# Image-Processing-Systems-Laboratory/DeepInPainting

Measured on AMD Instinct MI355X. Metric: train images/sec at 256x256, batch 8/GPU, 1/2/4/8 MI355X; IPSR layer ms, higher is better.
Workload: dtype f32; 1 GPU; BASELINE config 2: 256x256 synthetic images, 128x128 centre mask (M=256 of N=1024 feature positions), batch 8/GPU, fp32, full IPSR training step; global_batch=8, parallelism=dp1, dropout=True, conv_math=fp32, vgg16=seeded random init (no pretrained weights offline)

## Files before the change

### deepinpainting_amd/csrc/winograd.hip

```cpp
#include <type_traits>

#include "ipsr_common.h"

namespace ipsr {

typedef float f32x16 __attribute__((ext_vector_type(16)));
typedef const __attribute__((address_space(1))) void* gptr_t;
typedef __attribute__((address_space(3))) void* lptr_t;

constexpr int WG_BM = 128, WG_BN = 128, WG_BK = 16, WG_NBUF = 4, WG_THREADS = 256;

struct WinoSplit {
    int nsplit, sps, xi_split, nsplit_t, sps_t;
    int nxi = 36;
    __host__ __device__ int slabs() const { return xi_split >= nxi ? nsplit : (xi_split <= 0 ? nsplit_t : (nsplit > nsplit_t ? nsplit : nsplit_t)); }
    __host__ __device__ int of(int xi) const { return xi < xi_split ? nsplit : nsplit_t; }
    __host__ __device__ int head_xi() const { return xi_split < nxi ? xi_split : nxi; }
    __host__ int workgroups(int tiles_per_xi) const { return tiles_per_xi * (head_xi() * nsplit + (nxi - head_xi()) * nsplit_t); }
};

__device__ __forceinline__ void wino_load_sum(const float* __restrict__ M, const WinoSplit sp, size_t plane, size_t off, float m[6][6])
{
#pragma unroll
    for (int i = 0; i < 6; ++i)
// ... 1246 lines not shown
}

template <int IS, bool TMAJOR, int MODE, typename TIN>
__global__ void __launch_bounds__(256) wino5_window_kernel(const TIN* __restrict__ x, int B, int C, int H, int Wd, int nphase, int TY, int TX,
                                                           int Tp, int Cp, void* __restrict__ V, int remap)
{
    __shared__ __attribute__((aligned(16))) unsigned char smem[op_smem_bytes<TMAJOR, MODE>()];
    const int Ctot = nphase * C;
    const OpIdx ix = op_index<TMAJOR, MODE>(!TMAJOR && remap != 0);
    const int t = ix.t, cc = ix.c;
    if (!TMAJOR && MODE == 0 && t >= Tp) return;
    const int T = B * TY * TX;
    const bool live = t < T && cc < Ctot;
    int b = 0, ty = 0, tx = 0, ph = 0, c = 0;
    if (live) { b = t / (TY * TX); const int rem = t - b * TY * TX; ty = rem / TX; tx = rem - ty * TX; ph = cc / C; c = cc - ph * C; }
    const int offy = nphase == 4 ? (ph >> 1) - 1 : -1, offx = nphase == 4 ? (ph & 1) - 1 : -1;
    const TIN* xp = x + ((size_t)b * C + c) * H * Wd;
    float d[6][6];
#pragma unroll
    for (int i = 0; i < 6; ++i) {
        const int yy = IS * (5 * ty + i) + offy;
        const bool yok = live && (unsigned)yy < (unsigned)H;
#pragma unroll
        for (int j = 0; j < 6; ++j) {
            const int xx = IS * (5 * tx + j) + offx;
            d[i][j] = (yok && (unsigned)xx < (unsigned)Wd) ? ld1(xp, (size_t)yy * Wd + xx) : 0.0f;
        }
    }
    float w[6][6], v[6][6];
#pragma unroll
    for (int j = 0; j < 6; ++j) {
        const float col[6] = {d[0][j], d[1][j], d[2][j], d[3][j], d[4][j], d[5][j]};
        float o[6];
        wino_bt(col, o);
#pragma unroll
        for (int i = 0; i < 6; ++i) w[i][j] = o[i];
    }
#pragma unroll
    for (int i = 0; i < 6; ++i) wino_bt(w[i], v[i]);
    op_emit<TMAJOR, MODE>(smem, v, ix, V, TMAJOR ? Cp : Ctot, Tp);
}

__device__ __forceinline__ void wino_at5_2d(const float m[6][6], float o[5][5])
{
    float w[5][6];
#pragma unroll
    for (int j = 0; j < 6; ++j) {
        const float col[6] = {m[0][j], m[1][j], m[2][j], m[3][j], m[4][j], m[5][j]};
        float r5[5];
        wino_at5(col, r5);
#pragma unroll
        for (int i = 0; i < 5; ++i) w[i][j] = r5[i];
    }
#pragma unroll
    for (int i = 0; i < 5; ++i) wino_at5(w[i], o[i]);
}

template <typename TOUT>
__global__ void __launch_bounds__(256) wino5_output_kernel(const float* __restrict__ Mo, WinoSplit split, int B, int K, int Kp, int Ho, int Wo,
                                                           int TY, int TX, int Tp, TOUT* __restrict__ y)
{
    const int t = blockIdx.x * 256 + threadIdx.x, k = blockIdx.y;
    const int T = B * TY * TX;
    if (t >= T) return;
    float m[6][6], o[5][5];
    wino_load_sum(Mo, split, (size_t)Kp * Tp, (size_t)k * Tp + t, m);
    wino_at5_2d(m, o);
    const int b = t / (TY * TX), rem = t - b * TY * TX;
    const int ty = rem / TX, tx = rem - ty * TX;
    TOUT* yp = y + ((size_t)b * K + k) * Ho * Wo;
#pragma unroll
    for (int i = 0; i < 5; ++i)
#pragma unroll
        for (int j = 0; j < 5; ++j) {
            const int oy = 5 * ty + i, ox = 5 * tx + j;
            if (oy < Ho && ox < Wo) st1(yp, (size_t)oy * Wo + ox, o[i][j]);
        }
}

constexpr int W5R_TILES = 64;
template <typename TOUT>
__global__ void __launch_bounds__(256) wino5_output_rows_kernel(const float* __restrict__ Mo, WinoSplit split, int B, int K, int Kp, int nh, int nw,
                                                                int TY, int TX, int Tp, TOUT* __restrict__ y)
{
    __shared__ float blk[W5R_TILES][101];
    __shared__ int org_y[W5R_TILES], org_x[W5R_TILES], org_b[W5R_TILES];
    const int tl = threadIdx.x & 63, ph = threadIdx.x >> 6, ey = ph >> 1, ex = ph & 1;
    const int t0 = blockIdx.x * W5R_TILES, t = t0 + tl, k = blockIdx.y;
    const int T = B * TY * TX;
    if (t < T) {
        float m[6][6], o[5][5];
        wino_load_sum(Mo, split, (size_t)Kp * Tp, (size_t)(ph * K + k) * Tp + t, m);
        wino_at5_2d(m, o);
#pragma unroll
        for (int i = 0; i < 5; ++i)
#pragma unroll
            for (int j = 0; j < 5; ++j) blk[tl][(2 * i - ey + 1) * 10 + (2 * j - ex + 1)] = o[i][j];
        if (ph == 0) {
            const int b = t / (TY * TX), rem = t - b * TY * TX;
            const int ty = rem / TX, tx = rem - ty * TX;
            org_b[tl] = b; org_y[tl] = 10 * ty - 1; org_x[tl] = 10 * tx - 1;
        }
    }
    __syncthreads();
    const int Hy = 2 * nh, Wy = 2 * nw;
    const int ntile = min(W5R_TILES, T - t0);
    for (int e = threadIdx.x; e < 10 * 10 * W5R_TILES; e += 256) {
        const int r = e / (10 * W5R_TILES), xs = e - r * (10 * W5R_TILES);
        const int tile = xs / 10, c = xs - tile * 10;
        if (tile >= ntile) continue;
        const int fy = org_y[tile] + r, fx = org_x[tile] + c;
        if (fy < 0 || fy >= Hy || fx < 0 || fx >= Wy) continue;
        st1(y + ((size_t)org_b[tile] * K + k) * (size_t)Hy * Wy, (size_t)fy * Wy + fx, blk[tile][r * 10 + c]);
    }
}

template <int MODE, typename TIN>
__global__ void __launch_bounds__(256) wino_wrw_tile5_kernel(const TIN* __restrict__ dy, int B, int K, int Ho, int Wo, int TY, int TX,
                                                             int Tp, int Kp, void* __restrict__ Et)
{
    __shared__ __attribute__((aligned(16))) unsigned char smem[op_smem_bytes<true, MODE>()];
    const OpIdx ix = op_index<true, MODE>(false);
    const int t = ix.t, k = ix.c, T = B * TY * TX;
    const bool live = t < T && k < K;
    int b = 0, ty = 0, tx = 0;
    if (live) { b = t / (TY * TX); const int rem = t - b * TY * TX; ty = rem / TX; tx = rem - ty * TX; }
    const TIN* dp = dy + ((size_t)b * K + (live ? k : 0)) * Ho * Wo;
    float e[5][5];
#pragma unroll
    for (int i = 0; i < 5; ++i)
#pragma unroll
        for (int j = 0; j < 5; ++j) {
            const int yy = 5 * ty + i, xx = 5 * tx + j;
            e[i][j] = (live && yy < Ho && xx < Wo) ? ld1(dp, (size_t)yy * Wo + xx) : 0.0f;
        }
    float w[6][5], v[6][6];
#pragma unroll
    for (int j = 0; j < 5; ++j) {
        const float col[5] = {e[0][j], e[1][j], e[2][j], e[3][j], e[4][j]};
        float o[6];
        wino_g5(col, o);
#pragma unroll
        for (int i = 0; i < 6; ++i) w[i][j] = o[i];
    }
#pragma unroll
    for (int i = 0; i < 6; ++i) wino_g5(w[i], v[i]);
    op_emit<true, MODE>(smem, v, ix, Et, Kp, Tp);
}

__global__ void __launch_bounds__(256) wino_wrw_output2_kernel(const float* __restrict__ Mw, WinoSplit split, int Kc, int Cf, int Kp, int Cp,
                                                               float* __restrict__ dW)
{
    const int cf = blockIdx.x * 256 + threadIdx.x, kc = blockIdx.y, ph = blockIdx.z;
    if (cf >= Cf) return;
    float m[6][6], w[2][6], o[2][2];
    wino_load_sum(Mw, split, (size_t)Kp * Cp, (size_t)kc * Cp + (size_t)ph * Cf + cf, m);
#pragma unroll
    for (int j = 0; j < 6; ++j) {
        const float col[6] = {m[0][j], m[1][j], m[2][j], m[3][j], m[4][j], m[5][j]};
        float r2[2];
        wino_at2(col, r2);
        w[0][j] = r2[0]; w[1][j] = r2[1];
    }
    wino_at2(w[0], o[0]);
    wino_at2(w[1], o[1]);
    const int ey = ph >> 1, ex = ph & 1;
    float* dst = dW + ((size_t)kc * Cf + cf) * 16;
#pragma unroll
    for (int a = 0; a < 2; ++a)
#pragma unroll
        for (int b = 0; b < 2; ++b) dst[(2 * a + ey) * 4 + 2 * b + ex] = o[a][b];
}

struct S2Plan { int TY, TX, T, Tp, Kp, Cp, red; WinoSplit sp; size_t a_floats, b_floats, m_floats, total_bytes; };

static int s2_plan(int mode, int B, int Kc, int Cf, int nh, int nw, S2Plan* p, int math)
{
    if (mode < 0 || mode > 2) return fail(IPSR_ERR_INVALID, "4x4 stride-2 winograd: mode %d", mode);
    p->TY = mode == 1 ? (nh + 5) / 5 : (nh + 4) / 5;
    p->TX = mode == 1 ? (nw + 5) / 5 : (nw + 4) / 5;
    p->T = B * p->TY * p->TX;
    p->Tp = (p->T + WG_BN - 1) / WG_BN * WG_BN;
    size_t m1;
    if (mode == 2) {
        p->Kp = wino_rows_padded(Kc, math);
        p->Cp = (4 * Cf + WG_BN - 1) / WG_BN * WG_BN;
        p->red = p->Tp;
        p->a_floats = (size_t)36 * p->Tp * p->Kp * 3 / 2;
        p->b_floats = (size_t)36 * p->Tp * p->Cp * 3 / 2;
        m1 = (size_t)36 * p->Kp * p->Cp;
        p->sp = wino_choose_split(36 * wino_row_tiles(p->Kp) * (p->Cp / WG_BN), p->Tp / WG_BK, m1 * 4);
    } else {
        p->red = mode == 0 ? 4 * Cf : Kc;
        if (p->red % WG_BK != 0)
            return fail(IPSR_ERR_UNSUPPORTED, "4x4 stride-2 winograd: reduction length %d is not a multiple of %d", p->red, WG_BK);
        const int prod = mode == 0 ? Kc : 4 * Cf;
        p->Kp = wino_rows_padded(prod, math);
        p->Cp = p->red;
        p->a_floats = (size_t)36 * p->red * p->Kp * 3 / 2;
        p->b_floats = (size_t)36 * p->red * p->Tp * 3 / 2;
        m1 = (size_t)36 * p->Kp * p->Tp;
        p->sp = wino_choose_split(36 * wino_row_tiles(p->Kp) * (p->Tp / WG_BN), p->red / WG_BK, m1 * 4);
    }
    p->m_floats = m1 * p->sp.slabs();
    p->total_bytes = align_up(p->a_floats * 4, 256) + align_up(p->b_floats * 4, 256) + align_up(p->m_floats * 4, 256) + 256;
    return IPSR_OK;
}

size_t winograd_s2_ws_bytes(int mode, int B, int Kc, int Cf, int nh, int nw)
{
    S2Plan p, q;
    if (s2_plan(mode, B, Kc, Cf, nh, nw, &p, -1) != IPSR_OK || s2_plan(mode, B, Kc, Cf, nh, nw, &q, 0) != IPSR_OK) return 0;
    return p.total_bytes > q.total_bytes ? p.total_bytes : q.total_bytes;
}

int launch_winograd_s2(int mode, const void* a, const void* b2, void* out, int B, int Kc, int Cf, int nh, int nw,
                       void* ws, size_t ws_bytes, hipStream_t st, ConvArith ar = ConvArith{0, false, false})
{
    S2Plan p;
    if (int rc = s2_plan(mode, B, Kc, Cf, nh, nw, &p, ar.math)) return rc;
    if (ws_bytes < p.total_bytes) return fail(IPSR_ERR_WORKSPACE, "4x4 stride-2 winograd: workspace %zu < %zu", ws_bytes, p.total_bytes);
    if (!arith_ok(ar)) return fail(IPSR_ERR_INVALID, "4x4 stride-2 winograd: arithmetic %d", ar.math);
    if (ar.math && ((mode == 0 && Cf % 8 != 0) || (mode == 1 && (Cf % SPLIT_ROWS != 0 || p.Kp != 4 * Cf || Kc % 8 != 0)))) ar.math = 0;
    Carver cv(ws, ws_bytes);
    float* A = cv.take<float>(p.a_floats);
    float* Bv = cv.take<float>(p.b_floats);
    float* Mo = cv.take<float>(p.m_floats);
    const int remap = !debug_option(1);
    if (mode == 0 || mode == 1) {
        const float* w = static_cast<const float*>(b2);
        if (ar.math == 0) {
            if (mode == 0) wino52_filter_kernel<<<dim3(cdiv(p.Kp, 256), Cf), 256, 0, st>>>(w, Kc, Cf, p.Kp, 0, A);
            else wino52_filter_kernel<<<dim3(cdiv(Cf + (p.Kp - 4 * Cf), 256), Kc), 256, 0, st>>>(w, Kc, Cf, p.Kp, 1, A);
        } else {
            const dim3 fg = mode == 0 ? dim3(p.Kp / SPLIT_ROWS, Cf / 8) : dim3(Cf / SPLIT_ROWS, Kc / 8);
            if (ar.math == 2) wino52_filter_split_kernel<2><<<fg, 256, 0, st>>>(w, Kc, Cf, p.Kp, mode, reinterpret_cast<unsigned short*>(A));
            else wino52_filter_split_kernel<3><<<fg, 256, 0, st>>>(w, Kc, Cf, p.Kp, mode, reinterpret_cast<unsigned short*>(A));
        }
        with_mode(ar.math, [&](auto M) {
            constexpr int MODE = decltype(M)::value;
            with_type(ar.in_bf16, [&](auto* tag) {
                using T = ELEM_T(tag);
                if (mode == 0) wino5_window_kernel<2, false, MODE, T><<<op_grid(false, MODE, p.Tp, p.red), 256, 0, st>>>(static_cast<const T*>(a), B, Cf, 2 * nh, 2 * nw, 4, p.TY, p.TX, p.Tp, 0, Bv, remap);
                else wino5_window_kernel<1, false, MODE, T><<<op_grid(false, MODE, p.Tp, p.red), 256, 0, st>>>(static_cast<const T*>(a), B, Kc, nh, nw, 1, p.TY, p.TX, p.Tp, 0, Bv, remap);
            });
        });
        if (int rc = check_launch("wino5_window_kernel")) return rc;
        launch_wino_gemm(ar.math, A, Bv, p.red, p.Kp, p.Tp, p.sp, Mo, st, 72.0 * p.red * (mode == 0 ? Kc : 4 * Cf) * p.T);
        if (int rc = check_launch("wino_gemm_kernel")) return rc;
        with_type(ar.out_bf16, [&](auto* tag) {
            using T = ELEM_T(tag);
            if (mode == 0) wino5_output_kernel<T><<<dim3(cdiv(p.T, 256), Kc), 256, 0, st>>>(Mo, p.sp, B, Kc, p.Kp, nh, nw, p.TY, p.TX, p.Tp, static_cast<T*>(out));
            else wino5_output_rows_kernel<T><<<dim3(cdiv(p.T, W5R_TILES), Cf), 256, 0, st>>>(Mo, p.sp, B, Cf, p.Kp, nh, nw, p.TY, p.TX, p.Tp, static_cast<T*>(out));
        });
        return check_launch("wino5_output_kernel");
    }
    with_mode(ar.math, [&](auto M) {
        constexpr int MODE = decltype(M)::value;
        with_type(ar.in_bf16, [&](auto* tag) {
            using T = ELEM_T(tag);
            wino_wrw_tile5_kernel<MODE, T><<<op_grid(true, MODE, p.Tp, p.Kp), 256, 0, st>>>(static_cast<const T*>(b2), B, Kc, nh, nw, p.TY, p.TX, p.Tp, p.Kp, A);
            wino5_window_kernel<2, true, MODE, T><<<op_grid(true, MODE, p.Tp, p.Cp), 256, 0, st>>>(static_cast<const T*>(a), B, Cf, 2 * nh, 2 * nw, 4, p.TY, p.TX, p.Tp, p.Cp, Bv, 0);
        });
    });
    if (int rc = check_launch("wino5_window_kernel")) return rc;
    launch_wino_gemm(ar.math, A, Bv, p.Tp, p.Kp, p.Cp, p.sp, Mo, st, 72.0 * p.T * Kc * 4 * Cf);
    if (int rc = check_launch("wino_gemm_kernel")) return rc;
    wino_wrw_output2_kernel<<<dim3(cdiv(Cf, 256), Kc, 4), 256, 0, st>>>(Mo, p.sp, Kc, Cf, p.Kp, p.Cp, static_cast<float*>(out));
    return check_launch("wino_wrw_output2_kernel");
}

typedef float f32x4v __attribute__((ext_vector_type(4)));


__global__ void __launch_bounds__(256) sm_to_cn_kernel(const float* __restrict__ x, int B, int C, int HW, int Tp, float* __restrict__ out)
{
    const int n = blockIdx.x * 256 + threadIdx.x, c = blockIdx.y;
    if (n >= Tp) return;
    float v = 0.0f;
    if (n < B * HW) { const int b = n / HW, p = n - b * HW; v = x[((size_t)b * C + c) * HW + p]; }
    out[(size_t)c * Tp + n] = v;
}

__global__ void __launch_bounds__(256) sm_to_nc_kernel(const float* __restrict__ x, int B, int C, int HW, float* __restrict__ out)
{
    const int c = blockIdx.x * 256 + threadIdx.x, n = blockIdx.y;
    if (c >= C) return;
    float v = 0.0f;
    if (n < B * HW) { const int b = n / HW, p = n - b * HW; v = x[((size_t)b * C + c) * HW + p]; }
    out[(size_t)n * C + c] = v;
}

__device__ __forceinline__ float sm_tap(const float* __restrict__ f, int B, int C, int Hf, int Wf, int Ho, int Wo, int k, int st, int pad, int dil,
                                        int n, int col)
{
    if (n >= B * Ho * Wo) return 0.0f;
    const int kk = k * k;
    const int c = col / kk, t = col - c * kk, r = t / k, q = t - r * k;
    const int b = n / (Ho * Wo), o = n - b * Ho * Wo, oy = o / Wo, ox = o - oy * Wo;
    const int fy = oy * st - pad + r * dil, fx = ox * st - pad + q * dil;
    return ((unsigned)fy < (unsigned)Hf && (unsigned)fx < (unsigned)Wf) ? f[(((size_t)b * C + c) * Hf + fy) * Wf + fx] : 0.0f;
}

__global__ void __launch_bounds__(256) sm_im2col_nt_kernel(const float* __restrict__ f, int B, int C, int Hf, int Wf, int Ho, int Wo,
                                                           int k, int st, int pad, int dil, float* __restrict__ out)
{
    const int col = blockIdx.x * 256 + threadIdx.x, n = blockIdx.y;
    const int ncol = C * k * k;
    if (col >= ncol) return;
    out[(size_t)n * ncol + col] = sm_tap(f, B, C, Hf, Wf, Ho, Wo, k, st, pad, dil, n, col);
}

__global__ void __launch_bounds__(256) sm_im2col_cn_kernel(const float* __restrict__ f, int B, int C, int Hf, int Wf, int Ho, int Wo,
                                                           int k, int st, int pad, int dil, int Tp, float* __restrict__ out)
{
    const int n = blockIdx.x * 256 + threadIdx.x, col = blockIdx.y;
    if (n >= Tp) return;
    out[(size_t)col * Tp + n] = sm_tap(f, B, C, Hf, Wf, Ho, Wo, k, st, pad, dil, n, col);
}

__global__ void __launch_bounds__(256) sm_col2im_kernel(const float* __restrict__ M, int nslab, size_t slab_stride, int B, int C, int Hf, int Wf,
                                                        int Ho, int Wo, int k, int st, int pad, int dil, int Tp, float* __restrict__ out)
{
    const size_t idx = (size_t)blockIdx.x * 256 + threadIdx.x;
    const size_t total = (size_t)B * C * Hf * Wf;
    if (idx >= total) return;
    const int fx = (int)(idx % Wf), fy = (int)((idx / Wf) % Hf), c = (int)((idx / ((size_t)Wf * Hf)) % C), b = (int)(idx / ((size_t)Wf * Hf * C));
    float acc = 0.0f;
    for (int r = 0; r < k; ++r) {
        const int ny = fy + pad - r * dil;
        if (ny < 0 || ny % st) continue;
        const int oy = ny / st;
        if (oy >= Ho) continue;
        for (int q = 0; q < k; ++q) {
            const int nx = fx + pad - q * dil;
            if (nx < 0 || nx % st) continue;
            const int ox = nx / st;
            if (ox >= Wo) continue;
            const size_t off = (size_t)(c * k * k + r * k + q) * Tp + ((size_t)b * Ho + oy) * Wo + ox;
            for (int sl = 0; sl < nslab; ++sl) acc += M[(size_t)sl * slab_stride + off];
        }
    }
    out[idx] = acc;
}

__global__ void __launch_bounds__(256) sm_sum_to_nchw_kernel(const float* __restrict__ Y, int nslab, size_t slab_stride, int B, int R, int HW, int Tp,
                                                             float* __restrict__ out)
{
    const size_t idx = (size_t)blockIdx.x * 256 + threadIdx.x;
    if (idx >= (size_t)B * R * HW) return;
    const int o = (int)(idx % HW), r = (int)((idx / HW) % R), b = (int)(idx / ((size_t)HW * R));
    const size_t off = (size_t)r * Tp + (size_t)b * HW + o;
    float acc = 0.0f;
    for (int sl = 0; sl < nslab; ++sl) acc += Y[(size_t)sl * slab_stride + off];
    out[idx] = acc;
}

template <int NB>
__device__ __forceinline__ void sm_reduce4(f32x16 (&acc)[NB], float* lds, int wave, int lane)
{
    if (wave > 0) {
#pragma unroll
        for (int nb = 0; nb < NB; ++nb)
#pragma unroll
            for (int e = 0; e < 16; ++e) lds[(((wave - 1) * NB + nb) * 16 + e) * 64 + lane] = acc[nb][e];
    }
    __syncthreads();
    if (wave == 0) {
#pragma unroll
        for (int w = 0; w < 3; ++w)
#pragma unroll
            for (int nb = 0; nb < NB; ++nb)
#pragma unroll
                for (int e = 0; e < 16; ++e) acc[nb][e] += lds[((w * NB + nb) * 16 + e) * 64 + lane];
    }
    __syncthreads();
}

template <int NB>
__global__ void __launch_bounds__(256) sm_data_kernel(const float* __restrict__ Wm, const float* __restrict__ In, int R, int Q, int Tp, int rows_per_wave,
                                                      float* __restrict__ Mcol)
{
    __shared__ float red[3 * NB * 16 * 64];
    const int lane = threadIdx.x & 63, wave = __builtin_amdgcn_readfirstlane(threadIdx.x >> 6), m = lane & 31, h = lane >> 5;
    const int q0 = blockIdx.x * 128, n0 = blockIdx.z * (32 * NB);
    const int ra = min(R, (blockIdx.y * 4 + wave) * rows_per_wave), rb = min(R, ra + rows_per_wave);
    f32x16 acc[4][NB];
#pragma unroll
    for (int j = 0; j < 4; ++j)
#pragma unroll
        for (int nb = 0; nb < NB; ++nb)
#pragma unroll
            for (int e = 0; e < 16; ++e) acc[j][nb][e] = 0.0f;
    const float* wp = Wm + (size_t)(ra + h) * Q + q0 + 4 * m;
    const float* ip = In + (size_t)(ra + h) * Tp + n0 + m;
    constexpr int U = NB == 1 ? 8 : (NB == 2 ? 4 : 2);
    for (int r = ra; r < rb; r += 2 * U) {
        f32x4v a[U];
        float bv[U][NB];
#pragma unroll
        for (int u = 0; u < U; ++u) {
            const bool ok = r + 2 * u < rb;
            a[u] = ok ? *reinterpret_cast<const f32x4v*>(wp + (size_t)2 * u * Q) : f32x4v{0.0f, 0.0f, 0.0f, 0.0f};
#pragma unroll
            for (int nb = 0; nb < NB; ++nb) bv[u][nb] = ok ? ip[(size_t)2 * u * Tp + 32 * nb] : 0.0f;
        }
#pragma unroll
        for (int u = 0; u < U; ++u)
#pragma unroll
            for (int j = 0; j < 4; ++j)
#pragma unroll
                for (int nb = 0; nb < NB; ++nb) acc[j][nb] = __builtin_amdgcn_mfma_f32_32x32x2f32(a[u][j], bv[u][nb], acc[j][nb], 0, 0, 0);
        wp += (size_t)2 * U * Q;
        ip += (size_t)2 * U * Tp;
    }
    float* out = Mcol + (size_t)blockIdx.y * Q * Tp;
#pragma unroll
    for (int j = 0; j < 4; ++j) {
        sm_reduce4<NB>(acc[j], red, wave, lane);
        if (wave == 0) {
#pragma unroll
            for (int nb = 0; nb < NB; ++nb)
#pragma unroll
                for (int e = 0; e < 16; ++e) {
                    const int row = (e & 3) + 8 * (e >> 2) + 4 * h;
                    out[(size_t)(q0 + 4 * row + j) * Tp + n0 + 32 * nb + m] = acc[j][nb][e];
                }
        }
    }
}

template <int NB>
__global__ void __launch_bounds__(256) sm_fwd_kernel(const float* __restrict__ Wm, const float* __restrict__ Xc, int R, int Q, int Tp, int cols_per_wave,
                                                     float* __restrict__ Y)
{
    __shared__ float red[3 * NB * 16 * 64];
    const int lane = threadIdx.x & 63, wave = __builtin_amdgcn_readfirstlane(threadIdx.x >> 6), m = lane & 31, h = lane >> 5;
    const int r0 = blockIdx.x * 32, n0 = blockIdx.z * (32 * NB);
    const int qa = min(Q, (blockIdx.y * 4 + wave) * cols_per_wave), qb = min(Q, qa + cols_per_wave);
    f32x16 acc[NB];
#pragma unroll
    for (int nb = 0; nb < NB; ++nb)
#pragma unroll
        for (int e = 0; e < 16; ++e) acc[nb][e] = 0.0f;
    const float* wp = Wm + (size_t)(r0 + m) * Q + qa + 4 * h;
    const float* xp = Xc + (size_t)(qa + 4 * h) * Tp + n0 + m;
    constexpr int U = 4;
    for (int q = qa; q < qb; q += 8 * U) {
        f32x4v a[U];
        float bv[U][4][NB];
#pragma unroll
        for (int u = 0; u < U; ++u) {
            const bool ok = q + 8 * u < qb;
            a[u] = ok ? *reinterpret_cast<const f32x4v*>(wp + 8 * u) : f32x4v{0.0f, 0.0f, 0.0f, 0.0f};
#pragma unroll
            for (int j = 0; j < 4; ++j)
#pragma unroll
                for (int nb = 0; nb < NB; ++nb) bv[u][j][nb] = ok ? xp[(size_t)(8 * u + j) * Tp + 32 * nb] : 0.0f;
        }
#pragma unroll
        for (int u = 0; u < U; ++u)
#pragma unroll
            for (int j = 0; j < 4; ++j)
#pragma unroll
                for (int nb = 0; nb < NB; ++nb) acc[nb] = __builtin_amdgcn_mfma_f32_32x32x2f32(a[u][j], bv[u][j][nb], acc[nb], 0, 0, 0);
        wp += 8 * U;
        xp += (size_t)8 * U * Tp;
    }
    sm_reduce4<NB>(acc, red, wave, lane);
    if (wave == 0) {
        float* out = Y + (size_t)blockIdx.y * R * Tp;
#pragma unroll
        for (int nb = 0; nb < NB; ++nb)
#pragma unroll
            for (int e = 0; e < 16; ++e) {
                const int row = (e & 3) + 8 * (e >> 2) + 4 * h;
                out[(size_t)(r0 + row) * Tp + n0 + 32 * nb + m] = acc[nb][e];
            }
    }
}

__global__ void __launch_bounds__(64) sm_wrw_kernel(const float* __restrict__ Ct, const float* __restrict__ Vt, int R, int Q, int Pp, float* __restrict__ dW)
{
    const int lane = threadIdx.x, m = lane & 31, h = lane >> 5;
    const int q0 = blockIdx.x * 128, r0 = blockIdx.y * 32;
    f32x16 acc[4];
#pragma unroll
    for (int j = 0; j < 4; ++j)
#pragma unroll
        for (int e = 0; e < 16; ++e) acc[j][e] = 0.0f;
    const float* cp = Ct + (size_t)h * R + r0 + m;
    const float* vp = Vt + (size_t)h * Q + q0 + 4 * m;
    constexpr int U = 4;
    for (int p = 0; p < Pp; p += 2 * U) {
        float av[U];
        f32x4v b[U];
#pragma unroll
        for (int u = 0; u < U; ++u) {
            const bool ok = p + 2 * u < Pp;
            av[u] = ok ? cp[(size_t)2 * u * R] : 0.0f;
            b[u] = ok ? *reinterpret_cast<const f32x4v*>(vp + (size_t)2 * u * Q) : f32x4v{0.0f, 0.0f, 0.0f, 0.0f};
        }
#pragma unroll
        for (int u = 0; u < U; ++u)
#pragma unroll
            for (int j = 0; j < 4; ++j) acc[j] = __builtin_amdgcn_mfma_f32_32x32x2f32(av[u], b[u][j], acc[j], 0, 0, 0);
        cp += (size_t)2 * U * R;
        vp += (size_t)2 * U * Q;
    }
#pragma unroll
    for (int e = 0; e < 16; ++e) {
        const int row = (e & 3) + 8 * (e >> 2) + 4 * h;
        *reinterpret_cast<f32x4v*>(dW + (size_t)(r0 + row) * Q + q0 + 4 * m) = f32x4v{acc[0][e], acc[1][e], acc[2][e], acc[3][e]};
    }
}

struct SmPlan { int P, Tp, Pp, Q, nb, ngroups, nslab, per_slab; size_t a_floats, b_floats, m_floats, total_bytes; };

static int sm_plan(int op, int B, int R, int Cq, int Ho, int Wo, int Hf, int Wf, int k, int st, int pad, int dil, SmPlan* p)
{
    if (op < 0 || op > 2) return fail(IPSR_ERR_INVALID, "small-map convolution: op %d", op);
    if (k < 1 || k > 4 || st < 1 || st > 2 || dil < 1 || pad < 0) return fail(IPSR_ERR_UNSUPPORTED, "small-map convolution: k%d s%d p%d d%d", k, st, pad, dil);
    if (Ho != (Hf + 2 * pad - dil * (k - 1) - 1) / st + 1 || Wo != (Wf + 2 * pad - dil * (k - 1) - 1) / st + 1)
        return fail(IPSR_ERR_INVALID, "small-map convolution: %dx%d is not the output grid of %dx%d under k%d s%d p%d d%d", Ho, Wo, Hf, Wf, k, st, pad, dil);
    p->P = B * Ho * Wo;
    p->Q = Cq * k * k;
    if (p->Q % 128 != 0) return fail(IPSR_ERR_UNSUPPORTED, "small-map convolution: %d x %d taps is not a multiple of 128", Cq, k * k);
    if (R % 32 != 0) return fail(IPSR_ERR_UNSUPPORTED, "small-map convolution: %d weight rows are not a multiple of 32", R);
    if (p->P > 1024) return fail(IPSR_ERR_UNSUPPORTED, "small-map convolution: %d positions (made for <= 1024)", p->P);
    const int blocks = (p->P + 31) / 32;
    p->nb = blocks >= 4 ? 4 : (blocks == 3 ? 4 : blocks);
    if (op == 0 && p->nb == 4) p->nb = 2;
    p->ngroups = (blocks + p->nb - 1) / p->nb;
    p->Tp = p->ngroups * p->nb * 32;
    p->Pp = (p->P + 1) & ~1;
    p->a_floats = p->b_floats = p->m_floats = 0;
    p->nslab = 1; p->per_slab = 0;
    const size_t w_bytes = (size_t)R * p->Q * 4;
    if (op == 0) {
        const int qb = p->Q / 128;
        const size_t slab_bytes = (size_t)p->Q * p->Tp * 4;
        const int cap = (int)std::max<size_t>(1, w_bytes / slab_bytes);
        int ns = std::max(1, std::min({R / 64, cap, (256 + qb * p->ngroups - 1) / (qb * p->ngroups)}));
        p->per_slab = (((R + 4 * ns - 1) / (4 * ns)) + 1) & ~1;
        p->nslab = (R + 4 * p->per_slab - 1) / (4 * p->per_slab);
        p->b_floats = (size_t)R * p->Tp;
        p->m_floats = (size_t)p->nslab * p->Q * p->Tp;
    } else if (op == 2) {
        const int rb = R / 32;
        const size_t slab_bytes = (size_t)R * p->Tp * 4;
        const int cap = (int)std::max<size_t>(1, w_bytes / slab_bytes);
        int ns = std::max(1, std::min({p->Q / 256, cap, (256 + rb * p->ngroups - 1) / (rb * p->ngroups)}));
        p->per_slab = (((p->Q + 4 * ns - 1) / (4 * ns)) + 7) & ~7;
        p->nslab = (p->Q + 4 * p->per_slab - 1) / (4 * p->per_slab);
        p->b_floats = (size_t)p->Q * p->Tp;
        p->m_floats = (size_t)p->nslab * R * p->Tp;
    } else {
        p->a_floats = (size_t)p->Pp * R;
        p->b_floats = (size_t)p->Pp * p->Q;
    }
    p->total_bytes = align_up(p->a_floats * 4, 256) + align_up(p->b_floats * 4, 256) + align_up(p->m_floats * 4, 256) + 256;
    return IPSR_OK;
}

size_t smallmap_ws_bytes(int op, int B, int R, int Cq, int Ho, int Wo, int Hf, int Wf, int k, int st, int pad, int dil)
{
    SmPlan p;
    if (sm_plan(op, B, R, Cq, Ho, Wo, Hf, Wf, k, st, pad, dil, &p) != IPSR_OK) return 0;
    return p.total_bytes;
}

int launch_smallmap(int op, const float* a, const float* b2, float* out, int B, int R, int Cq, int Ho, int Wo, int Hf, int Wf,
                    int k, int st_, int pad, int dil, void* ws, size_t ws_bytes, hipStream_t st)
{
    SmPlan p;
    if (int rc = sm_plan(op, B, R, Cq, Ho, Wo, Hf, Wf, k, st_, pad, dil, &p)) return rc;
    if (ws_bytes < p.total_bytes) return fail(IPSR_ERR_WORKSPACE, "small-map convolution: workspace %zu < %zu", ws_bytes, p.total_bytes);
    Carver cv(ws, ws_bytes);
    float* A = cv.take<float>(p.a_floats);
    float* Bv = cv.take<float>(p.b_floats);
    float* Mo = cv.take<float>(p.m_floats);
    if (op == 0) {
        sm_to_cn_kernel<<<dim3(cdiv(p.Tp, 256), R), 256, 0, st>>>(a, B, R, Ho * Wo, p.Tp, Bv);
        const dim3 grid(p.Q / 128, p.nslab, p.ngroups);
        if (p.nb == 1) sm_data_kernel<1><<<grid, 256, 0, st>>>(b2, Bv, R, p.Q, p.Tp, p.per_slab, Mo);
        else sm_data_kernel<2><<<grid, 256, 0, st>>>(b2, Bv, R, p.Q, p.Tp, p.per_slab, Mo);
        if (int rc = check_launch("sm_data_kernel")) return rc;
        const size_t total = (size_t)B * Cq * Hf * Wf;
        sm_col2im_kernel<<<(unsigned)((total + 255) / 256), 256, 0, st>>>(Mo, p.nslab, (size_t)p.Q * p.Tp, B, Cq, Hf, Wf, Ho, Wo, k, st_, pad, dil, p.Tp, out);
        return check_launch("sm_col2im_kernel");
    }
    if (op == 2) {
        sm_im2col_cn_kernel<<<dim3(cdiv(p.Tp, 256), p.Q), 256, 0, st>>>(a, B, Cq, Hf, Wf, Ho, Wo, k, st_, pad, dil, p.Tp, Bv);
        const dim3 grid(R / 32, p.nslab, p.ngroups);
        if (p.nb == 1) sm_fwd_kernel<1><<<grid, 256, 0, st>>>(b2, Bv, R, p.Q, p.Tp, p.per_slab, Mo);
        else if (p.nb == 2) sm_fwd_kernel<2><<<grid, 256, 0, st>>>(b2, Bv, R, p.Q, p.Tp, p.per_slab, Mo);
        else sm_fwd_kernel<4><<<grid, 256, 0, st>>>(b2, Bv, R, p.Q, p.Tp, p.per_slab, Mo);
        if (int rc = check_launch("sm_fwd_kernel")) return rc;
        const size_t total = (size_t)B * R * Ho * Wo;
        sm_sum_to_nchw_kernel<<<(unsigned)((total + 255) / 256), 256, 0, st>>>(Mo, p.nslab, (size_t)R * p.Tp, B, R, Ho * Wo, p.Tp, out);
        return check_launch("sm_sum_to_nchw_kernel");
    }
    sm_to_nc_kernel<<<dim3(cdiv(R, 256), p.Pp), 256, 0, st>>>(a, B, R, Ho * Wo, A);
    sm_im2col_nt_kernel<<<dim3(cdiv(p.Q, 256), p.Pp), 256, 0, st>>>(b2, B, Cq, Hf, Wf, Ho, Wo, k, st_, pad, dil, Bv);
    sm_wrw_kernel<<<dim3(p.Q / 128, R / 32), 64, 0, st>>>(A, Bv, R, p.Q, p.Pp, out);
    return check_launch("sm_wrw_kernel");
}

}

using namespace ipsr;

extern "C" {

int ipsr_debug_force_wino_split(int nsplit, int xi_split, int nsplit_t)
{
    if (nsplit == 0 && xi_split == 0 && nsplit_t == 0) { g_force_split[0] = g_force_split[1] = g_force_split[2] = 0; return IPSR_OK; }
    if (nsplit < 1 || nsplit_t < 1 || xi_split < 1 || xi_split > 36) return fail(IPSR_ERR_INVALID, "ipsr_debug_force_wino_split: bad split %d,%d,%d", nsplit, xi_split, nsplit_t);
    g_force_split[0] = nsplit; g_force_split[1] = xi_split; g_force_split[2] = nsplit_t;
    return IPSR_OK;
}

int ipsr_wino_gemm_split(int rows, int cols, int reduction, int* out5)
{
    if (!out5 || rows < 1 || cols < 1 || reduction < 1 || rows % WG_BM || cols % WG_BN || reduction % WG_BK)
        return fail(IPSR_ERR_INVALID, "ipsr_wino_gemm_split: rows / cols must be multiples of 128 and the reduction of 16");
    const WinoSplit sp = wino_choose_split(36 * (rows / WG_BM) * (cols / WG_BN), reduction / WG_BK, (size_t)36 * rows * cols * 4);
    out5[0] = sp.nsplit; out5[1] = sp.sps; out5[2] = sp.xi_split; out5[3] = sp.nsplit_t; out5[4] = sp.sps_t;
    return IPSR_OK;
}

size_t ipsr_conv3x3_winograd_workspace_bytes(int op, int B, int Cin, int H, int W, int Cout)
{
    if (op < 0 || op > 3 || B < 1 || Cin < 1 || Cout < 1 || H < 1 || W < 1) return 0;
    const bool fwd = op == 0 || op == 2;
    return winograd_ws_bytes(B, fwd ? Cin : Cout, fwd ? Cout : Cin, H, W);
}

static int arith_from(const char* who, int math, int io, ConvArith* ar)
{
    if ((math != 0 && math != 2 && math != 3) || io < 0 || io > 3)
        return fail(IPSR_ERR_INVALID, "%s: math %d (0 = fp32 MFMA, 2 = split bf16 x3, 3 = split bf16 x6) / io %d (bit 0: bf16 activations in, bit 1: out)", who, math, io);
    ar->math = math; ar->in_bf16 = (io & 1) != 0; ar->out_bf16 = (io & 2) != 0;
    return IPSR_OK;
}

int ipsr_conv3x3_winograd_mp(int op, const void* in, const float* weight, const float* bias, int epilogue, float* filter_cache,
                             int filter_cache_valid, void* out, int B, int Cin, int H, int W, int Cout, int math, int io,
                             void* ws, size_t ws_bytes, void* stream)
{
    if (!in || !weight || !out || !ws) return fail(IPSR_ERR_INVALID, "ipsr_conv3x3_winograd: null pointer");
    if (op < 0 || op > 3 || B < 1 || Cin < 1 || Cout < 1 || H < 1 || W < 1) return fail(IPSR_ERR_INVALID, "ipsr_conv3x3_winograd: bad argument");
    if ((reinterpret_cast<uintptr_t>(ws) & 15u) || (reinterpret_cast<uintptr_t>(out) & 15u) || (reinterpret_cast<uintptr_t>(filter_cache) & 15u))
        return fail(IPSR_ERR_INVALID, "ipsr_conv3x3_winograd: out / workspace / filter_cache must be 16-byte aligned");
    ConvArith ar;
    if (int rc = arith_from("ipsr_conv3x3_winograd_mp", math, io, &ar)) return rc;
    if (reinterpret_cast<uintptr_t>(in) & (ar.in_bf16 ? 7u : 15u))
        return fail(IPSR_ERR_INVALID, "ipsr_conv3x3_winograd: in must be aligned to four elements");
    hipStream_t st = static_cast<hipStream_t>(stream);
    switch (op) {
        case 0:
            return launch_winograd(in, weight, out, B, Cin, Cout, H, W, 9, (long)Cin * 9, 0, ws, ws_bytes, st, bias, epilogue, filter_cache, filter_cache_valid, ar);
        case 1:
            return launch_winograd(in, weight, out, B, Cout, Cin, H, W, (long)Cin * 9, 9, 1, ws, ws_bytes, st, bias, epilogue, filter_cache, filter_cache_valid, ar);
        case 2:
            return launch_winograd(in, weight, out, B, Cin, Cout, H, W, (long)Cout * 9, 9, 1, ws, ws_bytes, st, bias, epilogue, filter_cache, filter_cache_valid, ar);
        default:
            return launch_winograd(in, weight, out, B, Cout, Cin, H, W, 9, (long)Cout * 9, 0, ws, ws_bytes, st, bias, epilogue, filter_cache, filter_cache_valid, ar);
    }
}

int ipsr_conv3x3_winograd(int op, const float* in, const float* weight, float* out, int B, int Cin, int H, int W, int Cout,
                          void* ws, size_t ws_bytes, void* stream)
{
    return ipsr_conv3x3_winograd_mp(op, in, weight, nullptr, 0, nullptr, 0, out, B, Cin, H, W, Cout, 0, 0, ws, ws_bytes, stream);
}

size_t ipsr_conv3x3_winograd_filter_floats(int op, int Cin, int Cout)
{
    if (op < 0 || op > 3 || Cin < 1 || Cout < 1) return 0;
    const bool fwd = op == 0 || op == 2;
    return winograd_filter_floats(fwd ? Cin : Cout, fwd ? Cout : Cin);
}

int ipsr_conv3x3_winograd_ex(int op, const float* in, const float* weight, const float* bias, int epilogue, float* filter_cache,
                             int filter_cache_valid, float* out, int B, int Cin, int H, int W, int Cout,
                             void* ws, size_t ws_bytes, void* stream)
{
    return ipsr_conv3x3_winograd_mp(op, in, weight, bias, epilogue, filter_cache, filter_cache_valid, out, B, Cin, H, W, Cout, 0, 0, ws, ws_bytes, stream);
}

size_t ipsr_conv4x4_winograd_workspace_bytes(int geom, int mode, int B, int Cin, int H, int W, int Cout)
{
    if (geom < 0 || geom > 1 || mode < 0 || mode > 2 || B < 1 || Cin < 1 || Cout < 1 || H < 2 || W < 2) return 0;
    return winograd_dil_ws_bytes(geom, mode, B, Cin, H, W, Cout);
}

int ipsr_conv4x4_winograd_mp(int geom, int mode, const void* a, const void* b, void* out, int B, int Cin, int H, int W, int Cout,
                             int math, int io, void* ws, size_t ws_bytes, void* stream)
{
    if (!a || !b || !out || !ws) return fail(IPSR_ERR_INVALID, "ipsr_conv4x4_winograd: null pointer");
    if (geom < 0 || geom > 1 || mode < 0 || mode > 2 || B < 1 || Cin < 1 || Cout < 1 || H < 2 || W < 2)
        return fail(IPSR_ERR_INVALID, "ipsr_conv4x4_winograd: bad argument");
    if ((reinterpret_cast<uintptr_t>(ws) & 15u) || (reinterpret_cast<uintptr_t>(out) & 15u))
        return fail(IPSR_ERR_INVALID, "ipsr_conv4x4_winograd: out / workspace must be 16-byte aligned");
    ConvArith ar;
    if (int rc = arith_from("ipsr_conv4x4_winograd_mp", math, io, &ar)) return rc;
    return launch_winograd_dil(geom, mode, a, b, out, B, Cin, H, W, Cout, ws, ws_bytes, static_cast<hipStream_t>(stream), ar);
}

int ipsr_conv4x4_winograd(int geom, int mode, const float* a, const float* b, float* out, int B, int Cin, int H, int W, int Cout,
                          void* ws, size_t ws_bytes, void* stream)
{
    return ipsr_conv4x4_winograd_mp(geom, mode, a, b, out, B, Cin, H, W, Cout, 0, 0, ws, ws_bytes, stream);
}

size_t ipsr_conv4x4_dilated_winograd_workspace_bytes(int mode, int B, int Cin, int H, int W, int Cout)
{
    return ipsr_conv4x4_winograd_workspace_bytes(0, mode, B, Cin, H, W, Cout);
}

int ipsr_conv4x4_dilated_winograd(int mode, const float* a, const float* b, float* out, int B, int Cin, int H, int W, int Cout,
                                  void* ws, size_t ws_bytes, void* stream)
{
    return ipsr_conv4x4_winograd(0, mode, a, b, out, B, Cin, H, W, Cout, ws, ws_bytes, stream);
}

size_t ipsr_conv4x4s2_winograd_workspace_bytes(int mode, int B, int Kc, int Cf, int nh, int nw)
{
    if (mode < 0 || mode > 2 || B < 1 || Kc < 1 || Cf < 1 || nh < 1 || nw < 1) return 0;
    return winograd_s2_ws_bytes(mode, B, Kc, Cf, nh, nw);
}

int ipsr_conv4x4s2_winograd_mp(int mode, const void* a, const void* b, void* out, int B, int Kc, int Cf, int nh, int nw,
                               int math, int io, void* ws, size_t ws_bytes, void* stream)
{
    if (!a || !b || !out || !ws) return fail(IPSR_ERR_INVALID, "ipsr_conv4x4s2_winograd: null pointer");
    if (mode < 0 || mode > 2 || B < 1 || Kc < 1 || Cf < 1 || nh < 1 || nw < 1) return fail(IPSR_ERR_INVALID, "ipsr_conv4x4s2_winograd: bad argument");
    if ((reinterpret_cast<uintptr_t>(ws) & 15u) || (reinterpret_cast<uintptr_t>(out) & 15u))
        return fail(IPSR_ERR_INVALID, "ipsr_conv4x4s2_winograd: out / workspace must be 16-byte aligned");
    if (mode != 2 && (reinterpret_cast<uintptr_t>(b) & 15u))
        return fail(IPSR_ERR_INVALID, "ipsr_conv4x4s2_winograd: the weight must be 16-byte aligned");
    ConvArith ar;
    if (int rc = arith_from("ipsr_conv4x4s2_winograd_mp", math, io, &ar)) return rc;
    return launch_winograd_s2(mode, a, b, out, B, Kc, Cf, nh, nw, ws, ws_bytes, static_cast<hipStream_t>(stream), ar);
}

int ipsr_conv4x4s2_winograd(int mode, const float* a, const float* b, float* out, int B, int Kc, int Cf, int nh, int nw,
                            void* ws, size_t ws_bytes, void* stream)
{
    return ipsr_conv4x4s2_winograd_mp(mode, a, b, out, B, Kc, Cf, nh, nw, 0, 0, ws, ws_bytes, stream);
}

size_t ipsr_conv_smallmap_workspace_bytes(int op, int B, int R, int Cq, int Ho, int Wo, int Hf, int Wf, int k, int stride, int pad, int dil)
{
    if (B < 1 || R < 1 || Cq < 1 || Ho < 1 || Wo < 1 || Hf < 1 || Wf < 1) return 0;
    return smallmap_ws_bytes(op, B, R, Cq, Ho, Wo, Hf, Wf, k, stride, pad, dil);
}

int ipsr_conv_smallmap(int op, const float* a, const float* b, float* out, int B, int R, int Cq, int Ho, int Wo, int Hf, int Wf,
                       int k, int stride, int pad, int dil, void* ws, size_t ws_bytes, void* stream)
{
    if (!a || !b || !out || !ws) return fail(IPSR_ERR_INVALID, "ipsr_conv_smallmap: null pointer");
    if (B < 1 || R < 1 || Cq < 1 || Ho < 1 || Wo < 1 || Hf < 1 || Wf < 1) return fail(IPSR_ERR_INVALID, "ipsr_conv_smallmap: bad argument");
    if ((reinterpret_cast<uintptr_t>(ws) & 15u) || (reinterpret_cast<uintptr_t>(out) & 15u) || (reinterpret_cast<uintptr_t>(a) & 15u) ||
        (reinterpret_cast<uintptr_t>(b) & 15u))
        return fail(IPSR_ERR_INVALID, "ipsr_conv_smallmap: operands / workspace must be 16-byte aligned");
    return launch_smallmap(op, a, b, out, B, R, Cq, Ho, Wo, Hf, Wf, k, stride, pad, dil, ws, ws_bytes, static_cast<hipStream_t>(stream));
}

size_t ipsr_conv3x3_winograd_wrw_workspace_bytes(int transposed, int B, int Cin, int H, int W, int Cout)
{
    if (B < 1 || Cin < 1 || Cout < 1 || H < 1 || W < 1) return 0;
    return transposed ? winograd_wrw_ws_bytes(B, Cin, Cout, H, W) : winograd_wrw_ws_bytes(B, Cout, Cin, H, W);
}

int ipsr_conv3x3_winograd_wrw_mp(int transposed, const void* x, const void* dy, float* dw, int B, int Cin, int H, int W, int Cout,
                                 int math, int io, void* ws, size_t ws_bytes, void* stream)
{
    if (!x || !dy || !dw || !ws) return fail(IPSR_ERR_INVALID, "ipsr_conv3x3_winograd_wrw: null pointer");
    if (B < 1 || Cin < 1 || Cout < 1 || H < 1 || W < 1) return fail(IPSR_ERR_INVALID, "ipsr_conv3x3_winograd_wrw: bad argument");
    if (reinterpret_cast<uintptr_t>(ws) & 15u) return fail(IPSR_ERR_INVALID, "ipsr_conv3x3_winograd_wrw: workspace must be 16-byte aligned");
    ConvArith ar;
    if (int rc = arith_from("ipsr_conv3x3_winograd_wrw_mp", math, io, &ar)) return rc;
    hipStream_t st = static_cast<hipStream_t>(stream);
    if (transposed) return launch_winograd_wrw(x, dy, dw, B, Cin, Cout, H, W, ws, ws_bytes, st, ar);
    return launch_winograd_wrw(dy, x, dw, B, Cout, Cin, H, W, ws, ws_bytes, st, ar);
}

int ipsr_conv3x3_winograd_wrw(int transposed, const float* x, const float* dy, float* dw, int B, int Cin, int H, int W, int Cout,
                              void* ws, size_t ws_bytes, void* stream)
{
    return ipsr_conv3x3_winograd_wrw_mp(transposed, x, dy, dw, B, Cin, H, W, Cout, 0, 0, ws, ws_bytes, stream);
}

}
```

Measured before the change: 344.1 images/sec.

## Fuse im2col/transpose prepasses into small-map conv GEMM kernels

The small-map convolution kernels (data-grad, forward, weight-grad) now gather operands directly from NCHW tensors with on-the-fly im2col addressing and precomputed tap masks, instead of running separate transpose/im2col kernels into workspace first. This removes extra kernel launches and a round trip through global memory for the materialized column matrices. In exchange, inner-loop loads become scattered, uncoalesced gathers with index arithmetic. The old prepass path is kept behind a debug option, and the weight-grad fusion is used only when there are at most 32 positions.

```diff
diff --git a/deepinpainting_amd/csrc/winograd.hip b/deepinpainting_amd/csrc/winograd.hip
--- a/deepinpainting_amd/csrc/winograd.hip
+++ b/deepinpainting_amd/csrc/winograd.hip
@@ -1572,6 +1572,30 @@
     return ((unsigned)fy < (unsigned)Hf && (unsigned)fx < (unsigned)Wf) ? f[(((size_t)b * C + c) * Hf + fy) * Wf + fx] : 0.0f;
 }
 
+struct SmGeo { int P, C, Hf, Wf, Ho, Wo, st, pad, dil; };
+
+template <int K>
+__device__ __forceinline__ void sm_position(const SmGeo& g, int n, int& base, unsigned& taps)
+{
+    base = 0; taps = 0u;
+    if (n >= g.P) return;
+    const int b = n / (g.Ho * g.Wo), o = n - b * g.Ho * g.Wo, oy = o / g.Wo, ox = o - oy * g.Wo;
+    const int fy0 = oy * g.st - g.pad, fx0 = ox * g.st - g.pad;
+    base = (b * g.C * g.Hf + fy0) * g.Wf + fx0;
+#pragma unroll
+    for (int r = 0; r < K; ++r)
+#pragma unroll
+        for (int q = 0; q < K; ++q)
+            if ((unsigned)(fy0 + r * g.dil) < (unsigned)g.Hf && (unsigned)(fx0 + q * g.dil) < (unsigned)g.Wf) taps |= 1u << (r * K + q);
+}
+
+template <int K>
+__device__ __forceinline__ float sm_gather(const float* __restrict__ f, const SmGeo& g, int base, unsigned taps, int col)
+{
+    const int c = col / (K * K), t = col - c * (K * K), r = t / K, q = t - r * K;
+    return ((taps >> t) & 1u) ? f[base + c * (g.Hf * g.Wf) + (r * g.Wf + q) * g.dil] : 0.0f;
+}
+
 __global__ void __launch_bounds__(256) sm_im2col_nt_kernel(const float* __restrict__ f, int B, int C, int Hf, int Wf, int Ho, int Wo,
                                                            int k, int st, int pad, int dil, float* __restrict__ out)
 {
@@ -1647,9 +1671,9 @@
     __syncthreads();
 }
 
-template <int NB>
+template <int NB, bool NCHW>
 __global__ void __launch_bounds__(256) sm_data_kernel(const float* __restrict__ Wm, const float* __restrict__ In, int R, int Q, int Tp, int rows_per_wave,
-                                                      float* __restrict__ Mcol)
+                                                      int P, int HW, float* __restrict__ Mcol)
 {
     __shared__ float red[3 * NB * 16 * 64];
     const int lane = threadIdx.x & 63, wave = __builtin_amdgcn_readfirstlane(threadIdx.x >> 6), m = lane & 31, h = lane >> 5;
@@ -1663,7 +1687,21 @@
 #pragma unroll
             for (int e = 0; e < 16; ++e) acc[j][nb][e] = 0.0f;
     const float* wp = Wm + (size_t)(ra + h) * Q + q0 + 4 * m;
-    const float* ip = In + (size_t)(ra + h) * Tp + n0 + m;
+    const size_t ldi = NCHW ? HW : Tp;
+    const float* ip[NB];
+    bool okn[NB];
+#pragma unroll
+    for (int nb = 0; nb < NB; ++nb) {
+        const int n = n0 + 32 * nb + m;
+        if (NCHW) {
+            const int b = n / HW;
+            okn[nb] = n < P;
+            ip[nb] = In + (okn[nb] ? ((size_t)b * R + ra + h) * HW + (n - b * HW) : 0);
+        } else {
+            okn[nb] = true;
+            ip[nb] = In + (size_t)(ra + h) * Tp + n;
+        }
+    }
     constexpr int U = NB == 1 ? 8 : (NB == 2 ? 4 : 2);
     for (int r = ra; r < rb; r += 2 * U) {
         f32x4v a[U];
@@ -1673,7 +1711,7 @@
             const bool ok = r + 2 * u < rb;
             a[u] = ok ? *reinterpret_cast<const f32x4v*>(wp + (size_t)2 * u * Q) : f32x4v{0.0f, 0.0f, 0.0f, 0.0f};
 #pragma unroll
-            for (int nb = 0; nb < NB; ++nb) bv[u][nb] = ok ? ip[(size_t)2 * u * Tp + 32 * nb] : 0.0f;
+            for (int nb = 0; nb < NB; ++nb) bv[u][nb] = (ok && okn[nb]) ? ip[nb][(size_t)2 * u * ldi] : 0.0f;
         }
 #pragma unroll
         for (int u = 0; u < U; ++u)
@@ -1682,7 +1720,8 @@
 #pragma unroll
                 for (int nb = 0; nb < NB; ++nb) acc[j][nb] = __builtin_amdgcn_mfma_f32_32x32x2f32(a[u][j], bv[u][nb], acc[j][nb], 0, 0, 0);
         wp += (size_t)2 * U * Q;
-        ip += (size_t)2 * U * Tp;
+#pragma unroll
+        for (int nb = 0; nb < NB; ++nb) ip[nb] += (size_t)2 * U * ldi;
     }
     float* out = Mcol + (size_t)blockIdx.y * Q * Tp;
 #pragma unroll
@@ -1700,9 +1739,9 @@
     }
 }
 
-template <int NB>
+template <int NB, int K>
 __global__ void __launch_bounds__(256) sm_fwd_kernel(const float* __restrict__ Wm, const float* __restrict__ Xc, int R, int Q, int Tp, int cols_per_wave,
-                                                     float* __restrict__ Y)
+                                                     SmGeo g, float* __restrict__ Y)
 {
     __shared__ float red[3 * NB * 16 * 64];
     const int lane = threadIdx.x & 63, wave = __builtin_amdgcn_readfirstlane(threadIdx.x >> 6), m = lane & 31, h = lane >> 5;
@@ -1715,6 +1754,12 @@
         for (int e = 0; e < 16; ++e) acc[nb][e] = 0.0f;
     const float* wp = Wm + (size_t)(r0 + m) * Q + qa + 4 * h;
     const float* xp = Xc + (size_t)(qa + 4 * h) * Tp + n0 + m;
+    int base[NB];
+    unsigned taps[NB];
+    if (K > 0) {
+#pragma unroll
+        for (int nb = 0; nb < NB; ++nb) sm_position<K ? K : 1>(g, n0 + 32 * nb + m, base[nb], taps[nb]);
+    }
     constexpr int U = 4;
     for (int q = qa; q < qb; q += 8 * U) {
         f32x4v a[U];
@@ -1726,7 +1771,10 @@
 #pragma unroll
             for (int j = 0; j < 4; ++j)
 #pragma unroll
-                for (int nb = 0; nb < NB; ++nb) bv[u][j][nb] = ok ? xp[(size_t)(8 * u + j) * Tp + 32 * nb] : 0.0f;
+                for (int nb = 0; nb < NB; ++nb) {
+                    if (K > 0) bv[u][j][nb] = ok ? sm_gather<K ? K : 1>(Xc, g, base[nb], taps[nb], q + 4 * h + 8 * u + j) : 0.0f;
+                    else bv[u][j][nb] = ok ? xp[(size_t)(8 * u + j) * Tp + 32 * nb] : 0.0f;
+                }
         }
 #pragma unroll
         for (int u = 0; u < U; ++u)
@@ -1750,7 +1798,9 @@
     }
 }
 
-__global__ void __launch_bounds__(64) sm_wrw_kernel(const float* __restrict__ Ct, const float* __restrict__ Vt, int R, int Q, int Pp, float* __restrict__ dW)
+template <int K>
+__global__ void __launch_bounds__(64) sm_wrw_kernel(const float* __restrict__ Ct, const float* __restrict__ Vt, int R, int Q, int Pp, SmGeo g,
+                                                    float* __restrict__ dW)
 {
     const int lane = threadIdx.x, m = lane & 31, h = lane >> 5;
     const int q0 = blockIdx.x * 128, r0 = blockIdx.y * 32;
@@ -1761,6 +1811,20 @@
         for (int e = 0; e < 16; ++e) acc[j][e] = 0.0f;
     const float* cp = Ct + (size_t)h * R + r0 + m;
     const float* vp = Vt + (size_t)h * Q + q0 + 4 * m;
+    int coff[4], rd[4], qd[4];
+    int pb = 0, poy = 0, pox = 0;
+    if (K > 0) {
+        constexpr int KK = K ? K : 1;
+#pragma unroll
+        for (int j = 0; j < 4; ++j) {
+            const int col = q0 + 4 * m + j, c = col / (KK * KK), t = col - c * (KK * KK), r = t / KK, q = t - r * KK;
+            rd[j] = r * g.dil; qd[j] = q * g.dil;
+            coff[j] = c * (g.Hf * g.Wf) + rd[j] * g.Wf + qd[j];
+        }
+        pb = h / (g.Ho * g.Wo);
+        poy = (h - pb * g.Ho * g.Wo) / g.Wo;
+        pox = h - (pb * g.Ho + poy) * g.Wo;
+    }
     constexpr int U = 4;
     for (int p = 0; p < Pp; p += 2 * U) {
         float av[U];
@@ -1768,6 +1832,19 @@
 #pragma unroll
         for (int u = 0; u < U; ++u) {
             const bool ok = p + 2 * u < Pp;
+            if (K > 0) {
+                const bool in = p + 2 * u + h < g.P;
+                av[u] = in ? Ct[((size_t)pb * R + r0 + m) * (g.Ho * g.Wo) + poy * g.Wo + pox] : 0.0f;
+                const int fy0 = poy * g.st - g.pad, fx0 = pox * g.st - g.pad;
+                const int base = (pb * g.C * g.Hf + fy0) * g.Wf + fx0;
+#pragma unroll
+                for (int j = 0; j < 4; ++j)
+                    b[u][j] = (in && (unsigned)(fy0 + rd[j]) < (unsigned)g.Hf && (unsigned)(fx0 + qd[j]) < (unsigned)g.Wf) ? Vt[base + coff[j]] : 0.0f;
+                pox += 2;
+                while (pox >= g.Wo) { pox -= g.Wo; ++poy; }
+                while (poy >= g.Ho) { poy -= g.Ho; ++pb; }
+                continue;
+            }
             av[u] = ok ? cp[(size_t)2 * u * R] : 0.0f;
             b[u] = ok ? *reinterpret_cast<const f32x4v*>(vp + (size_t)2 * u * Q) : f32x4v{0.0f, 0.0f, 0.0f, 0.0f};
         }
@@ -1783,6 +1860,15 @@
         const int row = (e & 3) + 8 * (e >> 2) + 4 * h;
         *reinterpret_cast<f32x4v*>(dW + (size_t)(r0 + row) * Q + q0 + 4 * m) = f32x4v{acc[0][e], acc[1][e], acc[2][e], acc[3][e]};
     }
+}
+
+template <typename F> static inline void with_ksize(int k, F&& f)
+{
+    if (k == 1) f(std::integral_constant<int, 1>{});
+    else if (k == 2) f(std::integral_constant<int, 2>{});
+    else if (k == 3) f(std::integral_constant<int, 3>{});
+    else if (k == 4) f(std::integral_constant<int, 4>{});
+    else f(std::integral_constant<int, 0>{});
 }
 
 struct SmPlan { int P, Tp, Pp, Q, nb, ngroups, nslab, per_slab; size_t a_floats, b_floats, m_floats, total_bytes; };
@@ -1850,30 +1936,44 @@
     float* A = cv.take<float>(p.a_floats);
     float* Bv = cv.take<float>(p.b_floats);
     float* Mo = cv.take<float>(p.m_floats);
+    const bool prepass = debug_option(2) == 1;
+    const bool prepass_wrw = prepass || (p.P > 32 && debug_option(2) != 2);
+    const SmGeo g{p.P, Cq, Hf, Wf, Ho, Wo, st_, pad, dil};
     if (op == 0) {
-        sm_to_cn_kernel<<<dim3(cdiv(p.Tp, 256), R), 256, 0, st>>>(a, B, R, Ho * Wo, p.Tp, Bv);
         const dim3 grid(p.Q / 128, p.nslab, p.ngroups);
-        if (p.nb == 1) sm_data_kernel<1><<<grid, 256, 0, st>>>(b2, Bv, R, p.Q, p.Tp, p.per_slab, Mo);
-        else sm_data_kernel<2><<<grid, 256, 0, st>>>(b2, Bv, R, p.Q, p.Tp, p.per_slab, Mo);
+        if (prepass) {
+            sm_to_cn_kernel<<<dim3(cdiv(p.Tp, 256), R), 256, 0, st>>>(a, B, R, Ho * Wo, p.Tp, Bv);
+            if (p.nb == 1) sm_data_kernel<1, false><<<grid, 256, 0, st>>>(b2, Bv, R, p.Q, p.Tp, p.per_slab, p.P, Ho * Wo, Mo);
+            else sm_data_kernel<2, false><<<grid, 256, 0, st>>>(b2, Bv, R, p.Q, p.Tp, p.per_slab, p.P, Ho * Wo, Mo);
+        } else if (p.nb == 1) sm_data_kernel<1, true><<<grid, 256, 0, st>>>(b2, a, R, p.Q, p.Tp, p.per_slab, p.P, Ho * Wo, Mo);
+        else sm_data_kernel<2, true><<<grid, 256, 0, st>>>(b2, a, R, p.Q, p.Tp, p.per_slab, p.P, Ho * Wo, Mo);
         if (int rc = check_launch("sm_data_kernel")) return rc;
         const size_t total = (size_t)B * Cq * Hf * Wf;
         sm_col2im_kernel<<<(unsigned)((total + 255) / 256), 256, 0, st>>>(Mo, p.nslab, (size_t)p.Q * p.Tp, B, Cq, Hf, Wf, Ho, Wo, k, st_, pad, dil, p.Tp, out);
         return check_launch("sm_col2im_kernel");
     }
     if (op == 2) {
-        sm_im2col_cn_kernel<<<dim3(cdiv(p.Tp, 256), p.Q), 256, 0, st>>>(a, B, Cq, Hf, Wf, Ho, Wo, k, st_, pad, dil, p.Tp, Bv);
         const dim3 grid(R / 32, p.nslab, p.ngroups);
-        if (p.nb == 1) sm_fwd_kernel<1><<<grid, 256, 0, st>>>(b2, Bv, R, p.Q, p.Tp, p.per_slab, Mo);
-        else if (p.nb == 2) sm_fwd_kernel<2><<<grid, 256, 0, st>>>(b2, Bv, R, p.Q, p.Tp, p.per_slab, Mo);
-        else sm_fwd_kernel<4><<<grid, 256, 0, st>>>(b2, Bv, R, p.Q, p.Tp, p.per_slab, Mo);
+        if (prepass) sm_im2col_cn_kernel<<<dim3(cdiv(p.Tp, 256), p.Q), 256, 0, st>>>(a, B, Cq, Hf, Wf, Ho, Wo, k, st_, pad, dil, p.Tp, Bv);
+        const float* x = prepass ? Bv : a;
+        with_ksize(prepass ? 0 : k, [&](auto KC) {
+            constexpr int K = decltype(KC)::value;
+            if (p.nb == 1) sm_fwd_kernel<1, K><<<grid, 256, 0, st>>>(b2, x, R, p.Q, p.Tp, p.per_slab, g, Mo);
+            else if (p.nb == 2) sm_fwd_kernel<2, K><<<grid, 256, 0, st>>>(b2, x, R, p.Q, p.Tp, p.per_slab, g, Mo);
+            else sm_fwd_kernel<4, K><<<grid, 256, 0, st>>>(b2, x, R, p.Q, p.Tp, p.per_slab, g, Mo);
+        });
         if (int rc = check_launch("sm_fwd_kernel")) return rc;
         const size_t total = (size_t)B * R * Ho * Wo;
         sm_sum_to_nchw_kernel<<<(unsigned)((total + 255) / 256), 256, 0, st>>>(Mo, p.nslab, (size_t)R * p.Tp, B, R, Ho * Wo, p.Tp, out);
         return check_launch("sm_sum_to_nchw_kernel");
     }
-    sm_to_nc_kernel<<<dim3(cdiv(R, 256), p.Pp), 256, 0, st>>>(a, B, R, Ho * Wo, A);
-    sm_im2col_nt_kernel<<<dim3(cdiv(p.Q, 256), p.Pp), 256, 0, st>>>(b2, B, Cq, Hf, Wf, Ho, Wo, k, st_, pad, dil, Bv);
-    sm_wrw_kernel<<<dim3(p.Q / 128, R / 32), 64, 0, st>>>(A, Bv, R, p.Q, p.Pp, out);
+    if (prepass_wrw) {
+        sm_to_nc_kernel<<<dim3(cdiv(R, 256), p.Pp), 256, 0, st>>>(a, B, R, Ho * Wo, A);
+        sm_im2col_nt_kernel<<<dim3(cdiv(p.Q, 256), p.Pp), 256, 0, st>>>(b2, B, Cq, Hf, Wf, Ho, Wo, k, st_, pad, dil, Bv);
+    }
+    with_ksize(prepass_wrw ? 0 : k, [&](auto KC) {
+        sm_wrw_kernel<decltype(KC)::value><<<dim3(p.Q / 128, R / 32), 64, 0, st>>>(prepass_wrw ? A : a, prepass_wrw ? Bv : b2, R, p.Q, p.Pp, g, out);
+    });
     return check_launch("sm_wrw_kernel");
 }
 
```

New measurement: 342.8 images/sec. About the same (-0.4%).
